# facebookresearch/PointContrast

Measured on AMD Instinct MI355X. Metric: scene-pairs/sec, ScanNet 2.5cm Res16UNet34C PointInfoNCE, higher is better.
Workload: dtype f32; 1 GPU; BASELINE configs[1]: Res16UNet34C, nce loss, voxel 0.025 m, 4 pairs/GPU, 87380+87371 active voxels per forward pair on rank 0, npos 4096, T 0.4, SGD(lr 0.1, mom 0.8, wd 1e-4); global_batch=4, parallelism=dp1, engine=native, pair_execution=one two-segment pass (BatchNorm statistics per cloud)

## Files before the change

pointcontrast_amd/csrc/common.h:

```cpp
#pragma once
#include <hip/hip_runtime.h>
#include <stdarg.h>
#include <stdint.h>
#include <stdio.h>

#include "../../include/pcmi.h"

namespace pcmi {

void set_error(const char* fmt, ...);

#define PCMI_HIP_CHECK(expr)                                                             \
  do {                                                                                   \
    hipError_t _e = (expr);                                                              \
    if (_e != hipSuccess) {                                                              \
      pcmi::set_error("%s:%d: %s -> %s", __FILE__, __LINE__, #expr, hipGetErrorString(_e)); \
      return PCMI_ERR_HIP;                                                               \
    }                                                                                    \
  } while (0)

#define PCMI_REQUIRE(cond, code, ...)  \
  do {                                 \
    if (!(cond)) {                     \
      pcmi::set_error(__VA_ARGS__);    \
      return (code);                   \
    }                                  \
  } while (0)

extern thread_local long g_launches;
#define PCMI_LAUNCH_CHECK()         \
  do {                              \
    ++pcmi::g_launches;             \
    PCMI_HIP_CHECK(hipGetLastError()); \
  } while (0)

static inline hipStream_t as_stream(pcmi_stream_t s) { return reinterpret_cast<hipStream_t>(s); }

static inline int64_t ceil_div(int64_t a, int64_t b) { return (a + b - 1) / b; }
static inline size_t align_up(size_t a, size_t b) { return (a + b - 1) / b * b; }

constexpr uint64_t kEmptyKey = ~0ull;
constexpr int kCoordBias = 1 << 17;

__host__ __device__ inline uint64_t pack_key(int b, int x, int y, int z) {
  return ((uint64_t)(uint32_t)b << 54) | ((uint64_t)(uint32_t)(x + kCoordBias) << 36) |
         ((uint64_t)(uint32_t)(y + kCoordBias) << 18) | (uint64_t)(uint32_t)(z + kCoordBias);
}

__host__ __device__ inline uint32_t hash_key(uint64_t k) {
  k ^= k >> 33;
  k *= 0xff51afd7ed558ccdull;
  k ^= k >> 33;
  k *= 0xc4ceb9fe1a85ec53ull;
  k ^= k >> 33;
  return (uint32_t)k;
}

#if defined(__HIPCC__)
__device__ inline bool arrive_last(unsigned* counter, unsigned expected, unsigned* s_flag ) {
  __syncthreads();
  if (threadIdx.x == 0 && threadIdx.y == 0 && threadIdx.z == 0) {
    __builtin_amdgcn_fence(__ATOMIC_RELEASE, "agent");
    asm volatile("s_waitcnt vmcnt(0)" ::: "memory");
    const unsigned t = __hip_atomic_fetch_add(counter, 1u, __ATOMIC_RELAXED, __HIP_MEMORY_SCOPE_AGENT);
    const unsigned last = (t + 1u == expected) ? 1u : 0u;
    if (last) {
      __hip_atomic_store(counter, 0u, __ATOMIC_RELAXED, __HIP_MEMORY_SCOPE_AGENT);
      __builtin_amdgcn_fence(__ATOMIC_ACQUIRE, "agent");
    }
    *s_flag = last;
  }
  __syncthreads();
  return *s_flag != 0u;
}
#endif

__host__ __device__ inline int floor_div(int a, int d) {
  int q = a / d;
  return (a % d != 0 && ((a < 0) != (d < 0))) ? q - 1 : q;
}

}
```

pointcontrast_amd/csrc/spconv.hip:

```cpp
#include <algorithm>
#include <cmath>
#include <cstdlib>

#include "common.h"
#include "internal.h"
#include "spconv_args.h"
#include "spconv_plan.h"

namespace pcmi {

typedef float f32x16 __attribute__((ext_vector_type(16)));
typedef float v4f __attribute__((ext_vector_type(4)));

constexpr int kKC = 32;


template <int NT, bool WT, int KC = kKC>
__device__ __forceinline__ void load_b_regs(v4f (&breg)[NT * KC / 32], const float* __restrict__ wb, int64_t w_sc,
                                            int64_t w_sn, int c0, int n0, int t) {
  constexpr int NS = 32 * NT;
#pragma unroll
  for (int i = 0; i < NT * KC / 32; ++i) {
    const int e = t + i * 256;
    if (!WT) {
// ... 180 lines not shown
#pragma unroll
            for (int nt = 0; nt < NT; ++nt) bf[q % PF][nt] = sb[(8 * (qq >> 2) + (qq & 3)) * LDB + nt * 32];
          }
          __builtin_amdgcn_sched_barrier(0);
        }
      }
      if (more) store_b((step + 1) & 1);
      __syncthreads();
#pragma unroll
      for (int b = 0; b < BPG; ++b) a0[b] = a1[b];
      v0 = v1;
    }
  }

  if (KG > 1) {
    if (kg > 0) {
      float* red = s_f + ((kg - 1) * RW + rg) * 32 * NS;
#pragma unroll
      for (int nt = 0; nt < NT; ++nt)
#pragma unroll
        for (int j = 0; j < 16; ++j) {
          const int i = (j & 3) + 8 * (j >> 2) + 4 * h;
          red[i * NS + nt * 32 + r] = acc[nt][j];
        }
    }
    __syncthreads();
    if (kg == 0) {
#pragma unroll
      for (int g = 1; g < KG; ++g) {
        const float* red = s_f + ((g - 1) * RW + rg) * 32 * NS;
#pragma unroll
        for (int nt = 0; nt < NT; ++nt)
#pragma unroll
          for (int j = 0; j < 16; ++j) {
            const int i = (j & 3) + 8 * (j >> 2) + 4 * h;
            acc[nt][j] += red[i * NS + nt * 32 + r];
          }
      }
    }
  }

  if (kg == 0) {
    float* outp = a.out + (PAIR ? 0 : (int64_t)blockIdx.z * a.split_stride);
    float bv[NT];
#pragma unroll
    for (int nt = 0; nt < NT; ++nt) bv[nt] = a.bias ? a.bias[n0 + nt * 32 + r] : 0.f;
#pragma unroll
    for (int j = 0; j < 16; ++j) {
      const int i = (j & 3) + 8 * (j >> 2) + 4 * h;
      const int32_t orow = s_orow[rg * 32 + i];
      if (orow >= 0) {
        float* op = outp + (int64_t)orow * a.out_ld + n0 + r;
        if (a.accumulate) {
#pragma unroll
          for (int nt = 0; nt < NT; ++nt) op[nt * 32] += acc[nt][j] + bv[nt];
        } else {
#pragma unroll
          for (int nt = 0; nt < NT; ++nt) op[nt * 32] = acc[nt][j] + bv[nt];
        }
      }
    }
  }
}

typedef float f32x4 __attribute__((ext_vector_type(4)));
__host__ __device__ constexpr int kConv16Waves(int nt) { return nt <= 3 ? 4 : 3; }

template <int NT, bool WT, bool SK>
__global__ __launch_bounds__(256, kConv16Waves(NT)) void spconv16p_kernel(ConvArgs a) {
  constexpr int TM = 128, NS = 32 * NT, CTN = 2 * NT;
  constexpr int LDB = NS + 4;
  constexpr int KSLOTS = PCMI_MAX_KERNEL_VOLUME;
  constexpr uint32_t kAbsent = 0x80000000u;
  constexpr int kRsrcFlags = 0x00020000;
  __shared__ __attribute__((aligned(16))) float s_f[2 * kKC * LDB];
  __shared__ uint32_t s_off[KSLOTS][TM];
  __shared__ int32_t s_orow[TM];
  __shared__ int2 s_kmeta[KSLOTS];
  __shared__ int32_t s_kabs[KSLOTS];
  __shared__ int32_t s_nk;
  __shared__ int64_t s_tile[2];

  const int n0 = blockIdx.y * NS;
  int sk_g = 0, sk_tile = 0, sk_u = 0, sk_u1 = 0;
  bool sk_first = true;
  if constexpr (SK) {
    const int G = (int)gridDim.x;
    sk_g = (int)(blockIdx.x & 7) * (G / 8) + (int)(blockIdx.x >> 3);
    const int U = a.sk_pref[a.sk_tiles] * (a.C / kKC);
    const int per = (U + G - 1) / G;
    sk_u = sk_g * per;
    sk_u1 = min(U, sk_u + per);
    if (sk_u >= sk_u1) return;
    if (threadIdx.x < 64) {
      int lo = 0, n = a.sk_tiles;
      while (n > 1) {
        const int stride = (n + 63) / 64;
        const int probe = lo + (int)threadIdx.x * stride;
        const bool le = probe < lo + n && a.sk_pref[probe] * (a.C / kKC) <= sk_u;
        const int cnt = __popcll(__ballot(le));
        const int nlo = lo + max(cnt - 1, 0) * stride;
        n = min(stride, lo + n - nlo);
        lo = nlo;
      }
      if (threadIdx.x == 0) s_tile[0] = lo;
    }
    __syncthreads();
    sk_tile = __builtin_amdgcn_readfirstlane((int)s_tile[0]);
  }
  const __amdgpu_buffer_rsrc_t xr = __builtin_amdgcn_make_buffer_rsrc(const_cast<float*>(a.x), 0, 0x7FFFFFFF, kRsrcFlags);
  const __amdgpu_buffer_rsrc_t wr = __builtin_amdgcn_make_buffer_rsrc(const_cast<float*>(a.w), 0, 0x7FFFFFFF, kRsrcFlags);
  const uint32_t ld_bytes = (uint32_t)(a.x_ld * 4);
  const uint32_t wk_bytes = (uint32_t)(a.w_kstride * 4);
  const int sk_total = SK ? sk_u1 - sk_u : 0;
  int sk_done = 0, prio_qtr = -1;
  for (;;) {
  bool sk_whole = true;
  int sk_next_u = 0, sk_c0 = 0, sk_steps = 0;
  int t = threadIdx.x;
  if constexpr (SK) asm volatile("" : "+v"(t));
  const int lane = t & 63, wave = t >> 6;
  const int i = lane & 15, kk = lane >> 4;
  if constexpr (SK) {
    const int64_t row0 = (int64_t)sk_tile * TM;
    const uint32_t tmask = a.sk_mask[sk_tile];
    const int nch_ = a.C / kKC;
    const int pref = a.sk_pref[sk_tile] * nch_, ns_t = __popc(tmask) * nch_;
    const int jb = sk_u - pref, je = min(sk_u1 - pref, ns_t);
    sk_whole = (jb == 0 && je == ns_t);
    sk_next_u = pref + je;
    const int o0 = jb / nch_, o1 = (je - 1) / nch_;
    sk_c0 = jb - o0 * nch_;
    sk_steps = je - jb;
    if (t < a.K && ((tmask >> t) & 1u)) {
      const int j = __popc(tmask & ((1u << t) - 1u));
      if (j >= o0 && j <= o1) {
        s_kabs[j - o0] = t;
        s_kmeta[j - o0] = make_int2(j - o0, (int)((uint32_t)a.wsel[t] * wk_bytes));
      }
    }
    if (t == 0) s_nk = sk_steps > 0 ? o1 - o0 + 1 : 0;
    if (t < TM) s_orow[t] = (row0 + t < a.n_rows) ? (a.perm ? a.perm[row0 + t] : (int32_t)(row0 + t)) : -1;
    __syncthreads();
    const int cnt = sk_steps > 0 ? o1 - o0 + 1 : 0;
    for (int p = t; p < cnt * TM; p += 256) {
      const int q = p / TM, rr = p - q * TM;
      const int64_t row = row0 + rr;
      const int32_t v = row < a.n_rows ? a.nbr[(int64_t)s_kabs[q] * a.n_rows + row] : -1;
      s_off[q][rr] = v >= 0 ? (uint32_t)v * ld_bytes : kAbsent;
    }
  } else {
    int64_t tile = blockIdx.x;
    if (a.xcd_tiles > 0) {
      tile = (int64_t)(blockIdx.x & 7) * a.xcd_tiles + (blockIdx.x >> 3);
      if (tile * TM >= a.n_rows) return;
    }
    const int64_t row0 = tile * TM;
    const int kbeg = (int)((int64_t)a.K * blockIdx.z / a.ksplit);
    const int kend = (int)((int64_t)a.K * (blockIdx.z + 1) / a.ksplit);
    if (t < TM) s_orow[t] = (row0 + t < a.n_rows) ? (a.perm ? a.perm[row0 + t] : (int32_t)(row0 + t)) : -1;
    for (int p = t; p < (kend - kbeg) * TM; p += 256) {
      const int q = p / TM, rr = p - q * TM;
      const int64_t row = row0 + rr;
      int32_t v = -1;
      if (row < a.n_rows) v = a.nbr ? a.nbr[(int64_t)(kbeg + q) * a.n_rows + row] : (int32_t)row;
      s_off[q][rr] = v >= 0 ? (uint32_t)v * ld_bytes : kAbsent;
    }
    __syncthreads();
    if (t < 64) {
      int nk = 0;
      for (int q = 0; q < kend - kbeg; ++q) {
        bool any = false;
        for (int rr = t; rr < TM; rr += 64) any |= (s_off[q][rr] != kAbsent);
        if (__any(any)) {
          if (t == 0) s_kmeta[nk] = make_int2(q, (int)((uint32_t)a.wsel[kbeg + q] * wk_bytes));
// ... 50 lines not shown
    const uint32_t wofs = (uint32_t)__builtin_amdgcn_readfirstlane(l_meta.y);
    const char* row = reinterpret_cast<const char*>(&s_off[0][0]) + min(krow, KSLOTS - 1) * (TM * 4) + off_lane;
    l_voff[0] = *reinterpret_cast<const uint32_t*>(row);
    l_voff[1] = *reinterpret_cast<const uint32_t*>(row + 64);
    const uint32_t soff = (uint32_t)__builtin_amdgcn_readfirstlane((int)(wofs + (uint32_t)lc * b_chunk_bytes));
#pragma unroll
    for (int q = 0; q < NT; ++q)
      breg[q] = __builtin_bit_cast(v4f, __builtin_amdgcn_raw_buffer_load_b128(wr, live ? bvo[q] : kAbsent, live ? soff : 0u, 0));
  };
  auto stage_a = [&](v4f (&dst)[2][2], bool live) -> int {
    const uint32_t v0 = live ? l_voff[0] : kAbsent, v1 = live ? l_voff[1] : kAbsent;
    const int va = (__any(v0 != kAbsent) ? 1 : 0) | (__any(v1 != kAbsent) ? 2 : 0);
    const uint32_t soff = (uint32_t)__builtin_amdgcn_readfirstlane(lc * (kKC * 4));
    const uint32_t o0 = v0 + 16 * kk, o1 = v1 + 16 * kk;
    dst[0][0] = __builtin_bit_cast(v4f, __builtin_amdgcn_raw_buffer_load_b128(xr, o0, soff, 0));
    dst[1][0] = __builtin_bit_cast(v4f, __builtin_amdgcn_raw_buffer_load_b128(xr, o1, soff, 0));
    dst[0][1] = __builtin_bit_cast(v4f, __builtin_amdgcn_raw_buffer_load_b128(xr, o0 + 64, soff, 0));
    dst[1][1] = __builtin_bit_cast(v4f, __builtin_amdgcn_raw_buffer_load_b128(xr, o1 + 64, soff, 0));
    return va;
  };

  if (nsteps > 0) {
    stage_meta();
    stage_b(true);
    va0 = stage_a(a0, true);
    store_b(0);
    __syncthreads();
    auto do_step = [&](int step, v4f (&cur)[2][2], int va_cur, v4f (&nxt)[2][2], int& va_nxt) {
      const bool more = step + 1 < nsteps;
      if constexpr (SK) {
        const int qtr = __builtin_amdgcn_readfirstlane(((sk_done + step) * 4) / max(sk_total, 1));
        if (qtr != prio_qtr) {
          prio_qtr = qtr;
          if (qtr <= 0) __builtin_amdgcn_s_setprio(3);
          else if (qtr == 1) __builtin_amdgcn_s_setprio(2);
          else if (qtr == 2) __builtin_amdgcn_s_setprio(1);
          else __builtin_amdgcn_s_setprio(0);
        }
      }
      const float* sb = s_f + (step & 1) * (kKC * LDB) + i + (4 * kk) * LDB;
      constexpr int QN = 8, PF = 2;
      float bf[PF][CTN];
      if (va_cur) {
#pragma unroll
        for (int q = 0; q < PF; ++q)
#pragma unroll
          for (int ct = 0; ct < CTN; ++ct) bf[q][ct] = sb[(16 * (q >> 2) + (q & 3)) * LDB + ct * 16];
      }
      __builtin_amdgcn_sched_barrier(0);
      const bool g0 = (va_cur & 1) != 0, g1 = (va_cur & 2) != 0;
#pragma unroll
      for (int q = 0; q < QN; ++q) {
        const float av0 = cur[0][q >> 2][q & 3], av1 = cur[1][q >> 2][q & 3];
        if (g0) {
#pragma unroll
          for (int ct = 0; ct < CTN; ++ct)
            acc[0][ct] = __builtin_amdgcn_mfma_f32_16x16x4f32(av0, bf[q % PF][ct], acc[0][ct], 0, 0, 0);
        }
        if (g1) {
#pragma unroll
          for (int ct = 0; ct < CTN; ++ct)
            acc[1][ct] = __builtin_amdgcn_mfma_f32_16x16x4f32(av1, bf[q % PF][ct], acc[1][ct], 0, 0, 0);
        }
        if (va_cur && q + PF < QN) {
          const int qq = q + PF;
#pragma unroll
          for (int ct = 0; ct < CTN; ++ct) bf[q % PF][ct] = sb[(16 * (qq >> 2) + (qq & 3)) * LDB + ct * 16];
        }
        if (q == 0) stage_meta();
        if (q == 1) stage_b(more);
        if (q == 2) va_nxt = stage_a(nxt, more);
        __builtin_amdgcn_sched_barrier(0);
      }
      if (more) store_b((step + 1) & 1);
      __syncthreads();
    };
    for (int step = 0; step < nsteps; step += 2) {
      do_step(step, a0, va0, a1, va1);
      if (step + 1 < nsteps) do_step(step + 1, a1, va1, a0, va0);
    }
  }

  if (SK && !sk_whole) {
    float* pp = a.sk_part + ((int64_t)(2 * sk_g + (sk_first ? 0 : 1)) * TM + wave * 32) * a.N + n0 + i;
#pragma unroll
    for (int g = 0; g < 2; ++g)
#pragma unroll
      for (int r = 0; r < 4; ++r) {
        const int rl = g * 16 + 4 * kk + r;
#pragma unroll
        for (int ct = 0; ct < CTN; ++ct) pp[(int64_t)rl * a.N + ct * 16] = acc[g][ct][r];
      }
  } else {
    float* outp = a.out + (int64_t)blockIdx.z * a.split_stride;
    float bv[CTN];
#pragma unroll
    for (int ct = 0; ct < CTN; ++ct) bv[ct] = a.bias ? a.bias[n0 + ct * 16 + i] : 0.f;
#pragma unroll
    for (int g = 0; g < 2; ++g)
#pragma unroll
      for (int r = 0; r < 4; ++r) {
        const int32_t orow = s_orow[wave * 32 + g * 16 + 4 * kk + r];
        if (orow >= 0) {
          float* op = outp + (int64_t)orow * a.out_ld + n0 + i;
          if (a.accumulate) {
#pragma unroll
            for (int ct = 0; ct < CTN; ++ct) op[ct * 16] += acc[g][ct][r] + bv[ct];
          } else {
#pragma unroll
            for (int ct = 0; ct < CTN; ++ct) op[ct * 16] = acc[g][ct][r] + bv[ct];
          }
        }
      }
  }
  if constexpr (!SK) {
    break;
  } else {
    sk_u = sk_next_u;
    ++sk_tile;
    sk_first = false;
    sk_done += nsteps;
    if (sk_u >= sk_u1) break;
    __syncthreads();
  }
  }
}

__global__ __launch_bounds__(256) void sk_fixup_kernel(const float* __restrict__ part, const int32_t* __restrict__ pref,
                                                       int n_tiles, int G, const int32_t* __restrict__ perm, int64_t n_rows,
                                                       int N, const float* __restrict__ bias, float* __restrict__ out,
                                                       int64_t out_ld, int accumulate, int sub) {
  constexpr int TM = 128;
  const int tile = blockIdx.x;
  const int U = pref[n_tiles] * sub, per = (U + G - 1) / G;
  const int u0 = pref[tile] * sub, u1 = pref[tile + 1] * sub;
  if (u1 <= u0) return;
  const int g_first = u0 / per, g_last = (u1 - 1) / per;
  if (g_first == g_last) return;
  const int n4 = N / 4;
  const int64_t row0 = (int64_t)tile * TM;
  for (int e = threadIdx.x; e < TM * n4; e += 256) {
    const int rr = e / n4, c = (e - rr * n4) * 4;
    const int64_t row = row0 + rr;
    if (row >= n_rows) continue;
    float4 sum = make_float4(0.f, 0.f, 0.f, 0.f);
    for (int g = g_first; g <= g_last; ++g) {
      const int slot = (u0 <= g * per) ? 0 : 1;
      const float4 v = *reinterpret_cast<const float4*>(part + ((int64_t)(2 * g + slot) * TM + rr) * N + c);
      sum.x += v.x;
      sum.y += v.y;
      sum.z += v.z;
      sum.w += v.w;
    }
    if (bias) {
      sum.x += bias[c];
      sum.y += bias[c + 1];
      sum.z += bias[c + 2];
      sum.w += bias[c + 3];
    }
    const int64_t orow = perm ? perm[row] : row;
    float4* dst = reinterpret_cast<float4*>(out + orow * out_ld + c);
    if (accumulate) {
      const float4 o = *dst;
      sum.x += o.x;
      sum.y += o.y;
      sum.z += o.z;
      sum.w += o.w;
    }
    *dst = sum;
  }
}

__global__ void split_reduce_kernel(const float* __restrict__ part, int64_t split_stride, int ksplit,
                                    int64_t n_rows, int N, const float* __restrict__ bias,
                                    float* __restrict__ out, int64_t out_ld, int accumulate) {
  const int64_t idx = (int64_t)blockIdx.x * blockDim.x + threadIdx.x;
  const int n4 = N / 4;
  if (idx >= n_rows * n4) return;
  const int64_t row = idx / n4;
  const int c = (int)(idx % n4) * 4;
  float4 s = make_float4(0.f, 0.f, 0.f, 0.f);
  for (int i0 = 0; i0 < ksplit; i0 += 8) {
    float4 v[8];
#pragma unroll
    for (int u = 0; u < 8; ++u)
      v[u] = i0 + u < ksplit ? *reinterpret_cast<const float4*>(part + (int64_t)(i0 + u) * split_stride + row * N + c)
                             : make_float4(0.f, 0.f, 0.f, 0.f);
#pragma unroll
    for (int u = 0; u < 8; ++u) {
      s.x += v[u].x;
      s.y += v[u].y;
      s.z += v[u].z;
      s.w += v[u].w;
    }
  }
  if (bias) {
    s.x += bias[c];
    s.y += bias[c + 1];
    s.z += bias[c + 2];
    s.w += bias[c + 3];
  }
  float4* dst = reinterpret_cast<float4*>(out + row * out_ld + c);
  if (accumulate) {
    const float4 o = *dst;
    s.x += o.x;
    s.y += o.y;
    s.z += o.z;
    s.w += o.w;
  }
  *dst = s;
}

template <int CIN>
__global__ __launch_bounds__(256) void stem_fwd_kernel(const float* __restrict__ x, int64_t x_ld,
                                                       const float* __restrict__ w, int cout,
                                                       const int32_t* __restrict__ nbr, int K,
                                                       int64_t n_rows, const float* __restrict__ bias,
                                                       float* __restrict__ out, int64_t out_ld) {
  extern __shared__ float s_w[];
  for (int i = threadIdx.x; i < K * CIN * cout; i += 256) s_w[i] = w[i];
  __syncthreads();
  const int rows_per_block = 256 / 32;
  const int n = threadIdx.x & 31;
  const int64_t row = (int64_t)blockIdx.x * rows_per_block + (threadIdx.x >> 5);
  if (row >= n_rows) return;
  for (int nn = n; nn < cout; nn += 32) {
    float acc = bias ? bias[nn] : 0.f;
    for (int k = 0; k < K; ++k) {
      const int32_t idx = nbr ? nbr[(int64_t)k * n_rows + row] : (int32_t)row;
      if (idx < 0) continue;
      const float* xp = x + (int64_t)idx * x_ld;
#pragma unroll
      for (int c = 0; c < CIN; ++c) acc = fmaf(xp[c], s_w[(k * CIN + c) * cout + nn], acc);
    }
    out[row * out_ld + nn] = acc;
  }
}

template <int K>
__global__ __launch_bounds__(256) void stem32_fwd_kernel(const float* __restrict__ x, int64_t x_ld,
                                                         const float* __restrict__ w ,
                                                         const int32_t* __restrict__ nbr, int64_t n_rows,
                                                         const float* __restrict__ bias, float* __restrict__ out,
                                                         int64_t out_ld) {
  const int64_t row = (int64_t)blockIdx.x * 256 + threadIdx.x;
  if (row >= n_rows) return;
  int32_t idx[K];
#pragma unroll
  for (int k = 0; k < K; ++k) idx[k] = nbr ? nbr[(int64_t)k * n_rows + row] : (int32_t)row;
  float xv[K][3];
#pragma unroll
  for (int k = 0; k < K; ++k) {
    const float* xp = x + (int64_t)max(idx[k], 0) * x_ld;
    const bool ok = idx[k] >= 0;
// ... 81 lines not shown
  const ConvPlan p = plan_conv(conv_env(), rows, 0, C, N, K, PCMI_CONV_FORM_TABLE);
  return p.kernel == PCMI_CONV_KERNEL_TABLE_X3 ? p.NT : 0;
}

static int run_gathered(const float* x, int64_t x_ld, int64_t x_rows, int C, const float* w, int cin, int cout,
                        bool w_transposed, int N, const pcmi_kmap_t* map, bool pair_mode,
                        bool swap_pairs, const int32_t* wsel, const float* bias, float* out,
                        int64_t out_ld, int64_t n_rows, int accumulate, void* ws, size_t ws_bytes,
                        hipStream_t st) {
  PCMI_REQUIRE(C % 32 == 0 && N % 32 == 0, PCMI_ERR_UNSUPPORTED,
               "spconv: channels (%d -> %d) must be multiples of 32 on the MFMA path", C, N);
  PCMI_REQUIRE(x_ld % 4 == 0 && out_ld >= N && out_ld % 4 == 0 && ((uintptr_t)x % 16 == 0) && ((uintptr_t)w % 16 == 0) &&
                   ((uintptr_t)out % 16 == 0),
               PCMI_ERR_INVALID, "spconv: operands must be 16-byte aligned with ld %% 4 == 0");
  if (n_rows == 0) return PCMI_OK;
  ConvArgs a = {};
  a.x = x;
  a.x_ld = x_ld;
  a.C = C;
  a.w = w;
  a.w_kstride = (int64_t)cin * cout;
  if (!w_transposed) {
    a.w_sc = cout;
    a.w_sn = 1;
  } else {
    a.w_sc = 1;
    a.w_sn = cout;
  }
  a.N = N;
  a.K = map ? map->K : 1;
  for (int k = 0; k < PCMI_MAX_KERNEL_VOLUME; ++k) a.wsel[k] = wsel ? wsel[k] : k;
  a.n_rows = n_rows;
  a.bias = bias;
  a.nbr = !map || pair_mode ? nullptr : map->nbr;
  a.ksplit = 1;
  a.accumulate = accumulate;
  a.out = out;
  a.out_ld = out_ld;
  int form = !map ? PCMI_CONV_FORM_NONE : pair_mode ? PCMI_CONV_FORM_PAIRS : PCMI_CONV_FORM_TABLE;
  if (form == PCMI_CONV_FORM_TABLE && map->perm && map->nbr_perm) {
    a.nbr = map->nbr_perm;
    a.perm = map->perm;
    if (map->tile_pref && map->n_tiles == ceil_div(n_rows, 128)) form = PCMI_CONV_FORM_TABLE_UNITS;
  }
  const ConvPlan p = plan_conv(conv_env(), n_rows, x_rows * x_ld * 4, C, N, a.K, form);
  PCMI_REQUIRE(p.ws_bytes == 0 || (ws && ws_bytes >= p.ws_bytes), PCMI_ERR_WORKSPACE, "spconv: workspace %zu < %zu bytes",
               ws_bytes, p.ws_bytes);
  const int terms = conv_terms();
  if (p.pack_bytes) {
    a.wpack = x3_find_prepacked(w, w_transposed, p.NT, terms);
    if (!a.wpack) {
      a.wpack = (char*)ws + p.pack_offset;
      const int rc_pack = x3_pack_weights(a, p.NT, const_cast<void*>(a.wpack), st, terms);
      if (rc_pack) return rc_pack;
    }
  }
  int rc;
  switch (p.kernel) {
    case PCMI_CONV_KERNEL_PAIR: {
      a.pair_src = swap_pairs ? map->pair_in : map->pair_out;
      a.pair_dst = swap_pairs ? map->pair_out : map->pair_in;
      a.offs = map->offs;
      const int TM = 32 * p.RW;
      int64_t tiles = 0;
      if (map->M >= 0)
        for (int k = 0; k < a.K; ++k) tiles += ceil_div(map->offs_host[k + 1] - map->offs_host[k], TM);
      else
        tiles = ceil_div(kmap_pairs_bound(*map), TM) + a.K;
      if (tiles == 0) return PCMI_OK;
      dim3 grid((unsigned)tiles, (unsigned)(N / (32 * p.NT)), 1);
      return w_transposed ? launch_rw<true, true>(p.RW, p.NT, a, grid, st) : launch_rw<false, true>(p.RW, p.NT, a, grid, st);
    }
    case PCMI_CONV_KERNEL_32R:
      return conv32r_launch(w_transposed, a, st);
    case PCMI_CONV_KERNEL_UNITS_16:
    case PCMI_CONV_KERNEL_UNITS_X3: {
      const bool x3 = p.kernel == PCMI_CONV_KERNEL_UNITS_X3;
      const int G = x3 ? x3_workgroups(p.NT, terms) : sk_workgroups(p.NT);
      a.sk_mask = map->tile_mask;
      a.sk_pref = map->tile_pref;
      a.sk_tiles = (int)map->n_tiles;
      a.sk_part = (float*)ws;
      dim3 grid((unsigned)G, (unsigned)(N / (32 * p.NT)), 1);
      if (x3)
        rc = x3_launch(p.NT, true, a, grid, st, terms);
      else
        rc = w_transposed ? launch16<true, true>(p.NT, a, grid, st) : launch16<false, true>(p.NT, a, grid, st);
      if (rc) return rc;
      const int sub = C / kKC;
      sk_fixup_kernel<<<dim3((unsigned)a.sk_tiles), 256, 0, st>>>(a.sk_part, a.sk_pref, a.sk_tiles, G, a.perm, n_rows, N, bias,
                                                                out, out_ld, accumulate, sub);
      PCMI_LAUNCH_CHECK();
      return PCMI_OK;
    }
  }
  if (p.ksplit > 1) {
    a.ksplit = p.ksplit;
    a.split_stride = n_rows * N;
    a.out = (float*)ws;
    a.out_ld = N;
    a.bias = nullptr;
    a.accumulate = 0;
  }
  int64_t tiles = ceil_div(n_rows, 32 * p.RW);
  if (tiles >= 64) {
    a.xcd_tiles = (int)ceil_div(tiles, 8);
    tiles = (int64_t)a.xcd_tiles * 8;
  }
  dim3 grid((unsigned)tiles, (unsigned)(N / (32 * p.NT)), (unsigned)p.ksplit);
  switch (p.kernel) {
    case PCMI_CONV_KERNEL_TABLE_X3: rc = x3_launch(p.NT, false, a, grid, st, terms); break;
    case PCMI_CONV_KERNEL_TABLE_16:
      rc = w_transposed ? launch16<true, false>(p.NT, a, grid, st) : launch16<false, false>(p.NT, a, grid, st);
      break;
    case PCMI_CONV_KERNEL_DEEP: rc = w_transposed ? launch_deep<true>(p.NT, a, grid, st) : launch_deep<false>(p.NT, a, grid, st); break;
    default: rc = w_transposed ? launch_rw<true, false>(p.RW, p.NT, a, grid, st) : launch_rw<false, false>(p.RW, p.NT, a, grid, st);
  }
  if (rc) return rc;
  if (p.ksplit > 1) {
    const int64_t n4 = n_rows * (N / 4);
    split_reduce_kernel<<<dim3((unsigned)ceil_div(n4, 256)), 256, 0, st>>>((const float*)ws, a.split_stride, p.ksplit,
                                                                         n_rows, N, bias, out, out_ld, accumulate);
    PCMI_LAUNCH_CHECK();
  }
  return PCMI_OK;
}

size_t spconv_fwd_bwd_workspace(int64_t n_in, int64_t n_out, int cin, int cout, int K) {
  const ConvEnv env = conv_env();
  auto split = [&](int64_t rows, int C, int N) -> size_t {
    if (rows <= 0 || C % 32 != 0 || N % 32 != 0) return 0;
    return std::max(plan_conv(env, rows, 0, C, N, K, PCMI_CONV_FORM_TABLE).split_bytes,
                    plan_conv(env, rows, INT64_MAX, C, N, K, PCMI_CONV_FORM_TABLE).split_bytes);
  };
  const size_t ks = std::max(split(n_out, cin, cout), split(n_in, cout, cin));
  const size_t sk = n_in == n_out ? std::max(sk_partial_bytes(env, n_out, cout, K), sk_partial_bytes(env, n_in, cin, K)) : 0;
  const size_t pack = (K > 1 && cin % 32 == 0 && cout % 32 == 0) ? x3_pack_bytes(K, cin, cout) : 0;
  return align_up(std::max(ks, sk), 256) + pack;
}

}

namespace pcmi {

int spconv_forward_m32(const float* in, int64_t in_ld, int64_t n_in, int cin, const float* weight, int cout,
                       const pcmi_kmap_t* map, int transpose, const float* bias, float* out, int64_t out_ld,
                       int64_t n_out, int accumulate, void* ws, size_t ws_bytes, hipStream_t st) {
  PCMI_REQUIRE(in && weight && out && cin > 0 && cout > 0, PCMI_ERR_INVALID, "spconv_fwd: null/empty argument");
  if (map) {
    const int64_t mi = transpose ? map->n_out : map->n_in, mo = transpose ? map->n_in : map->n_out;
    PCMI_REQUIRE(mi == n_in && mo == n_out, PCMI_ERR_INVALID, "spconv_fwd: rows (%lld -> %lld) do not match the map (%lld -> %lld)",
                 (long long)n_in, (long long)n_out, (long long)mi, (long long)mo);
  } else {
    PCMI_REQUIRE(n_in == n_out, PCMI_ERR_INVALID, "spconv_fwd: dense path needs n_in == n_out");
  }
  if (cin < 8) {
    PCMI_REQUIRE(cin == 3 && !transpose && !accumulate && (!map || map->stride == 1), PCMI_ERR_UNSUPPORTED,
                 "spconv_fwd: cin=%d only supported as the 3-channel stride-1 stem", cin);
    if (n_out == 0) return PCMI_OK;
    const int K = map ? map->K : 1;
    if (cout == 32 && K == 27 && out_ld % 4 == 0 && (uintptr_t)out % 16 == 0) {
      stem32_fwd_kernel<27><<<dim3((unsigned)ceil_div(n_out, 256)), 256, 0, st>>>(in, in_ld, weight, map->nbr, n_out, bias, out,
                                                                                 out_ld);
      PCMI_LAUNCH_CHECK();
      return PCMI_OK;
    }
    const size_t lds = sizeof(float) * K * 3 * cout;
    stem_fwd_kernel<3><<<dim3((unsigned)ceil_div(n_out, 8)), 256, lds, st>>>(in, in_ld, weight, cout, map ? map->nbr : nullptr,
                                                                            K, n_out, bias, out, out_ld);
    PCMI_LAUNCH_CHECK();
    return PCMI_OK;
  }
  const bool pair_mode = map && transpose;
  PCMI_REQUIRE(!(map && transpose && map->stride != 2), PCMI_ERR_UNSUPPORTED, "spconv_fwd: transposed conv needs a stride-2 map");
  return run_gathered(in, in_ld, n_in, cin, weight, cin, cout, false, cout, map, pair_mode, false, nullptr, bias, out,
                      out_ld, n_out, accumulate, ws, ws_bytes, st);
// ... 74 lines not shown
```

pointcontrast_amd/csrc/spconv_args.h:

```cpp
#pragma once
#include "common.h"

namespace pcmi {

struct ConvArgs {
  const float* x;
  int64_t x_ld;
  int C;
  const float* w;
  int64_t w_kstride;
  int64_t w_sc, w_sn;
  int N;
  const int32_t* nbr;
  const int32_t* perm;
  const int32_t* pair_src;
  const int32_t* pair_dst;
  const int64_t* offs;
  int K;
  int32_t wsel[PCMI_MAX_KERNEL_VOLUME];
  int64_t n_rows;
  float* out;
  int64_t out_ld;
  int64_t split_stride;
  int ksplit;
  const float* bias;
  int xcd_tiles;
  int accumulate;
  const uint32_t* sk_mask;
  const int32_t* sk_pref;
  int sk_tiles;
  float* sk_part;
  const void* wpack;
};

size_t x3_pack_bytes(int K, int C, int N);
int x3_pack_weights(const ConvArgs& a, int NT, void* out, hipStream_t st, int terms);
int x3_launch(int NT, bool sk, const ConvArgs& a, dim3 grid, hipStream_t st, int terms);
int x3_workgroups(int NT, int terms);
int x3_plan_nt(int64_t rows, int C, int N, int K);

bool conv32r_eligible(int64_t min_rows, int64_t rows, int64_t x_bytes, int C, int N, int K, bool table);
int conv32r_launch(bool w_transposed, const ConvArgs& a, hipStream_t st);

struct X3PackJob {
  const float* w;
  int64_t w_kstride, w_sc, w_sn;
  int K, C, N, NS;
  int terms;
  void* out;
  int64_t first_item;
};
int x3_pack_many(const X3PackJob* jobs_dev, int n_jobs, int64_t total_items, hipStream_t st, int64_t first_item = 0);
struct X3Prepacked {
  const float* w;
  int transposed;
  int NT;
  int terms;
  const void* pack;
};
void x3_set_prepacked(const X3Prepacked* table, int n);
const void* x3_find_prepacked(const float* w, bool transposed, int NT, int terms);

}
```

pointcontrast_amd/csrc/spconv_x3.hip:

```cpp
#include <algorithm>
#include <cstdio>
#include <cstdlib>

#include "common.h"
#include "internal.h"
#include "spconv_args.h"
#include "x3_split.h"

namespace pcmi {

__host__ __device__ constexpr int x3_piece(int n, int kk) { return (n >> 4) * 64 + kk * 16 + (n & 15); }

__host__ __device__ constexpr int x3_channel(int kk, int e) { return 4 * kk + (e & 3) + 16 * (e >> 2); }

template <int TERMS>
__global__ __launch_bounds__(256) void x3_pack_kernel(const float* __restrict__ w, int64_t w_kstride, int64_t w_sc, int64_t w_sn,
                                                      int K, int C, int N, int NS, u32x4* __restrict__ out) {
  const int nch = C / kKC, nns = N / NS;
  const int64_t total = (int64_t)K * nch * nns * NS * 4;
  const int64_t idx = (int64_t)blockIdx.x * 256 + threadIdx.x;
  if (idx >= total) return;
  const int kk = (int)(idx & 3);
  int64_t r = idx >> 2;
  const int nl = (int)(r % NS);
// ... 7 lines not shown
#pragma unroll
  for (int e = 0; e < 4; ++e) {
    x0[e] = wb[(int64_t)(cc * kKC + x3_channel(kk, e)) * w_sc];
    x1[e] = wb[(int64_t)(cc * kKC + x3_channel(kk, e + 4)) * w_sc];
  }
  u32x4 h, m, l;
  split_terms<TERMS>(x0, x1, h, m, l);
  u32x4* blk = out + (((int64_t)wk * nch + cc) * nns + ns) * (TERMS * NS * 4);
  const int piece = x3_piece(nl, kk);
  blk[0 * NS * 4 + piece] = h;
  if constexpr (TERMS == 3) {
    blk[1 * NS * 4 + piece] = m;
    blk[2 * NS * 4 + piece] = l;
  }
}

__global__ __launch_bounds__(256) void x3_pack_many_kernel(const X3PackJob* __restrict__ jobs, int n_jobs, int64_t total,
                                                           int64_t item0) {
  const int64_t idx = item0 + (int64_t)blockIdx.x * 256 + threadIdx.x;
  if (idx >= total) return;
  int lo = 0, hi = n_jobs - 1;
  while (lo < hi) {
    const int mid = (lo + hi + 1) >> 1;
    if (jobs[mid].first_item <= idx) lo = mid; else hi = mid - 1;
  }
  const X3PackJob jb = jobs[lo];
  const int64_t loc = idx - jb.first_item;
  const int nch = jb.C / kKC, nns = jb.N / jb.NS;
  const int kk = (int)(loc & 3);
  int64_t r = loc >> 2;
  const int nl = (int)(r % jb.NS);
  r /= jb.NS;
  const int ns = (int)(r % nns);
  r /= nns;
  const int cc = (int)(r % nch);
  const int wk = (int)(r / nch);
  const float* wb = jb.w + (int64_t)wk * jb.w_kstride + (int64_t)(ns * jb.NS + nl) * jb.w_sn;
  v4f x0, x1;
#pragma unroll
  for (int e = 0; e < 4; ++e) {
    x0[e] = wb[(int64_t)(cc * kKC + x3_channel(kk, e)) * jb.w_sc];
    x1[e] = wb[(int64_t)(cc * kKC + x3_channel(kk, e + 4)) * jb.w_sc];
  }
  const int piece = x3_piece(nl, kk);
  if (jb.terms == 1) {
    u32x4 h;
    split1(x0, x1, h);
    reinterpret_cast<u32x4*>(jb.out)[(((int64_t)wk * nch + cc) * nns + ns) * (jb.NS * 4) + piece] = h;
    return;
  }
  u32x4 h, m, l;
  split3(x0, x1, h, m, l);
  u32x4* blk = reinterpret_cast<u32x4*>(jb.out) + (((int64_t)wk * nch + cc) * nns + ns) * (3 * jb.NS * 4);
  blk[0 * jb.NS * 4 + piece] = h;
  blk[1 * jb.NS * 4 + piece] = m;
  blk[2 * jb.NS * 4 + piece] = l;
}

template <int TERMS>
constexpr int x3_min_waves(int NT) { return TERMS == 3 ? (NT == 4 ? 2 : 3) : (NT == 2 ? 4 : 3); }
template <int NT, bool SK, bool DMA, int TERMS>
__global__ __launch_bounds__(256, x3_min_waves<TERMS>(NT)) void spconv16x_kernel(ConvArgs a) {
  constexpr int TM = 128, NS = 32 * NT, CTN = 2 * NT;
  constexpr int KSLOTS = PCMI_MAX_KERNEL_VOLUME;
  constexpr uint32_t kAbsent = 0x80000000u;
  constexpr int kRsrcFlags = 0x00020000;
  constexpr int PIECES = TERMS * NS * 4;
  constexpr int BLOCK_BYTES = PIECES * 16;
  constexpr int BR = (PIECES + 255) / 256;
  static_assert(CTN >= 3, "the three load stages sit behind the MFMAs of column tiles 0, 1, 2");
  __shared__ __attribute__((aligned(16))) u32x4 s_b[2][PIECES];
  __shared__ uint32_t s_off[KSLOTS][TM];
  __shared__ int32_t s_orow[TM];
  __shared__ int2 s_kmeta[KSLOTS];
  __shared__ int32_t s_kabs[KSLOTS];
  __shared__ int32_t s_nk;
  __shared__ int64_t s_tile[2];

  const int n0 = blockIdx.y * NS;
  const int nch = a.C / kKC;
  const uint32_t chunk_bytes = (uint32_t)gridDim.y * BLOCK_BYTES;
  const uint32_t wk_bytes = (uint32_t)nch * chunk_bytes;
  const uint32_t slice_bytes = (uint32_t)blockIdx.y * BLOCK_BYTES;
  int sk_g = 0, sk_tile = 0, sk_u = 0, sk_u1 = 0;
  bool sk_first = true;
  if constexpr (SK) {
    const int G = (int)gridDim.x;
    sk_g = (int)(blockIdx.x & 7) * (G / 8) + (int)(blockIdx.x >> 3);
    const int U = a.sk_pref[a.sk_tiles] * nch;
    const int per = (U + G - 1) / G;
    sk_u = sk_g * per;
    sk_u1 = min(U, sk_u + per);
    if (sk_u >= sk_u1) return;
    if (threadIdx.x < 64) {
      int lo = 0, n = a.sk_tiles;
      while (n > 1) {
        const int stride = (n + 63) / 64;
        const int probe = lo + (int)threadIdx.x * stride;
        const bool le = probe < lo + n && a.sk_pref[probe] * nch <= sk_u;
        const int cnt = __popcll(__ballot(le));
        const int nlo = lo + max(cnt - 1, 0) * stride;
        n = min(stride, lo + n - nlo);
        lo = nlo;
      }
      if (threadIdx.x == 0) s_tile[0] = lo;
    }
    __syncthreads();
    sk_tile = __builtin_amdgcn_readfirstlane((int)s_tile[0]);
  }
  const __amdgpu_buffer_rsrc_t xr = __builtin_amdgcn_make_buffer_rsrc(const_cast<float*>(a.x), 0, 0x7FFFFFFF, kRsrcFlags);
  const __amdgpu_buffer_rsrc_t wr = __builtin_amdgcn_make_buffer_rsrc(const_cast<void*>(a.wpack), 0, 0x7FFFFFFF, kRsrcFlags);
  const uint32_t ld_bytes = (uint32_t)(a.x_ld * 4);
  const int sk_total = SK ? sk_u1 - sk_u : 0;
  int sk_done = 0, prio_qtr = -1;
  for (;;) {
  bool sk_whole = true;
  int sk_next_u = 0, sk_c0 = 0, sk_steps = 0;
  int t = threadIdx.x;
  if constexpr (SK) asm volatile("" : "+v"(t));
  const int lane = t & 63, wave = t >> 6;
  const int i = lane & 15, kk = lane >> 4;
  if constexpr (SK) {
    const int64_t row0 = (int64_t)sk_tile * TM;
    const uint32_t tmask = a.sk_mask[sk_tile];
    const int pref = a.sk_pref[sk_tile] * nch, ns_t = __popc(tmask) * nch;
    const int jb = sk_u - pref, je = min(sk_u1 - pref, ns_t);
    sk_whole = (jb == 0 && je == ns_t);
    sk_next_u = pref + je;
    const int o0 = jb / nch, o1 = (je - 1) / nch;
    sk_c0 = jb - o0 * nch;
    sk_steps = je - jb;
    if (t < a.K && ((tmask >> t) & 1u)) {
      const int j = __popc(tmask & ((1u << t) - 1u));
      if (j >= o0 && j <= o1) {
        s_kabs[j - o0] = t;
        s_kmeta[j - o0] = make_int2(j - o0, (int)((uint32_t)a.wsel[t] * wk_bytes + slice_bytes));
      }
    }
    if (t == 0) s_nk = sk_steps > 0 ? o1 - o0 + 1 : 0;
    if (t < TM) s_orow[t] = (row0 + t < a.n_rows) ? (a.perm ? a.perm[row0 + t] : (int32_t)(row0 + t)) : -1;
    __syncthreads();
    const int cnt = sk_steps > 0 ? o1 - o0 + 1 : 0;
    {
      const int rr = t & (TM - 1);
      const int64_t row = row0 + rr;
      const bool row_ok = row < a.n_rows;
      const int64_t row_c = row_ok ? row : a.n_rows - 1;
      for (int q0 = t >> 7; q0 < cnt; q0 += 8) {
        int32_t v[4];
#pragma unroll
        for (int u = 0; u < 4; ++u) v[u] = a.nbr[(int64_t)s_kabs[min(q0 + 2 * u, cnt - 1)] * a.n_rows + row_c];
#pragma unroll
        for (int u = 0; u < 4; ++u)
          if (q0 + 2 * u < cnt) s_off[q0 + 2 * u][rr] = (row_ok && v[u] >= 0) ? (uint32_t)v[u] * ld_bytes : kAbsent;
      }
    }
  } else {
    int64_t tile = blockIdx.x;
    if (a.xcd_tiles > 0) {
      tile = (int64_t)(blockIdx.x & 7) * a.xcd_tiles + (blockIdx.x >> 3);
      if (tile * TM >= a.n_rows) return;
    }
    const int64_t row0 = tile * TM;
    const int kbeg = (int)((int64_t)a.K * blockIdx.z / a.ksplit);
    const int kend = (int)((int64_t)a.K * (blockIdx.z + 1) / a.ksplit);
    if (t < TM) s_orow[t] = (row0 + t < a.n_rows) ? (a.perm ? a.perm[row0 + t] : (int32_t)(row0 + t)) : -1;
    for (int p = t; p < (kend - kbeg) * TM; p += 256) {
      const int q = p / TM, rr = p - q * TM;
      const int64_t row = row0 + rr;
      int32_t v = -1;
      if (row < a.n_rows) v = a.nbr ? a.nbr[(int64_t)(kbeg + q) * a.n_rows + row] : (int32_t)row;
      s_off[q][rr] = v >= 0 ? (uint32_t)v * ld_bytes : kAbsent;
    }
    __syncthreads();
    if (t < 64) {
// ... 87 lines not shown
    dst[1][1] = __builtin_bit_cast(v4f, __builtin_amdgcn_raw_buffer_load_b128(xr, o1 + 64, soff, 0));
    return va;
  };

  if (nsteps > 0) {
    stage_meta();
    stage_b(true, 0);
    va0 = stage_a(a0, true);
    store_b(0);
    __syncthreads();
    auto do_step = [&](int step, v4f (&cur)[2][2], int va_cur, v4f (&nxt)[2][2], int& va_nxt) {
      const bool more = step + 1 < nsteps;
      if constexpr (SK) {
        const int qtr = __builtin_amdgcn_readfirstlane(((sk_done + step) * 4) / max(sk_total, 1));
        if (qtr != prio_qtr) {
          prio_qtr = qtr;
          if (qtr <= 0) __builtin_amdgcn_s_setprio(3);
          else if (qtr == 1) __builtin_amdgcn_s_setprio(2);
          else if (qtr == 2) __builtin_amdgcn_s_setprio(1);
          else __builtin_amdgcn_s_setprio(0);
        }
      }
      const bool g0 = (va_cur & 1) != 0, g1 = (va_cur & 2) != 0;
      u32x4 ah[2], am[2], al[2];
      if (g0) split_terms<TERMS>(cur[0][0], cur[0][1], ah[0], am[0], al[0]);
      if (g1) split_terms<TERMS>(cur[1][0], cur[1][1], ah[1], am[1], al[1]);
      const u32x4* sb = &s_b[step & 1][kk * 16 + i];
      u32x4 bh[2], bm[2], bl[2];
      if (va_cur) {
        bh[0] = sb[0 * NS * 4];
        if constexpr (TERMS == 3) {
          bm[0] = sb[1 * NS * 4];
          bl[0] = sb[2 * NS * 4];
        }
      }
      __builtin_amdgcn_sched_barrier(0);
#pragma unroll
      for (int ct = 0; ct < CTN; ++ct) {
        const int rb = ct & 1;
        if (va_cur && ct + 1 < CTN) {
          bh[rb ^ 1] = sb[(0 * NS + 16 * (ct + 1)) * 4];
          if constexpr (TERMS == 3) {
            bm[rb ^ 1] = sb[(1 * NS + 16 * (ct + 1)) * 4];
            bl[rb ^ 1] = sb[(2 * NS + 16 * (ct + 1)) * 4];
          }
        }
#define PCMI_X3_MFMA(G, AT, BT)                                                                                             \
  acc[G][ct] = __builtin_amdgcn_mfma_f32_16x16x32_bf16(__builtin_bit_cast(bf16x8, AT[G]), __builtin_bit_cast(bf16x8, BT[rb]), \
                                                       acc[G][ct], 0, 0, 0)
#define PCMI_X3_SIX(G)        \
  if constexpr (TERMS == 3) { \
    PCMI_X3_MFMA(G, al, bh);  \
    PCMI_X3_MFMA(G, ah, bl);  \
    PCMI_X3_MFMA(G, am, bm);  \
    PCMI_X3_MFMA(G, am, bh);  \
    PCMI_X3_MFMA(G, ah, bm);  \
  }                           \
  PCMI_X3_MFMA(G, ah, bh)
        if (g0 && g1) {
          PCMI_X3_SIX(0);
          PCMI_X3_SIX(1);
        } else if (g0) {
          PCMI_X3_SIX(0);
        } else if (g1) {
          PCMI_X3_SIX(1);
        }
#undef PCMI_X3_SIX
#undef PCMI_X3_MFMA
        if (ct == 0) stage_meta();
        if (ct == 1) stage_b(more, (step + 1) & 1);
        if (ct == 2) va_nxt = stage_a(nxt, more);
        __builtin_amdgcn_sched_barrier(0);
      }
      if (more) store_b((step + 1) & 1);
      __syncthreads();
    };
    for (int step = 0; step < nsteps; step += 2) {
      do_step(step, a0, va0, a1, va1);
      if (step + 1 < nsteps) do_step(step + 1, a1, va1, a0, va0);
    }
  }

  if (SK && !sk_whole) {
    float* pp = a.sk_part + ((int64_t)(2 * sk_g + (sk_first ? 0 : 1)) * TM + wave * 32) * a.N + n0 + i;
#pragma unroll
    for (int g = 0; g < 2; ++g)
#pragma unroll
      for (int r = 0; r < 4; ++r) {
        const int rl = g * 16 + 4 * kk + r;
#pragma unroll
        for (int ct = 0; ct < CTN; ++ct) pp[(int64_t)rl * a.N + ct * 16] = acc[g][ct][r];
      }
  } else {
    float* outp = a.out + (int64_t)blockIdx.z * a.split_stride;
    float bv[CTN];
#pragma unroll
    for (int ct = 0; ct < CTN; ++ct) bv[ct] = a.bias ? a.bias[n0 + ct * 16 + i] : 0.f;
#pragma unroll
    for (int g = 0; g < 2; ++g)
#pragma unroll
      for (int r = 0; r < 4; ++r) {
        const int32_t orow = s_orow[wave * 32 + g * 16 + 4 * kk + r];
        if (orow >= 0) {
          float* op = outp + (int64_t)orow * a.out_ld + n0 + i;
          if (a.accumulate) {
#pragma unroll
            for (int ct = 0; ct < CTN; ++ct) op[ct * 16] += acc[g][ct][r] + bv[ct];
          } else {
#pragma unroll
            for (int ct = 0; ct < CTN; ++ct) op[ct * 16] = acc[g][ct][r] + bv[ct];
          }
        }
      }
  }
  if constexpr (!SK) {
    break;
  } else {
    sk_u = sk_next_u;
    ++sk_tile;
    sk_first = false;
    sk_done += nsteps;
    if (sk_u >= sk_u1) break;
    __syncthreads();
  }
  }
}

template <bool SK, bool DMA, int TERMS>
static int launch_x3(int NT, const ConvArgs& a, dim3 grid, hipStream_t st) {
  switch (NT) {
    case 2: spconv16x_kernel<2, SK, DMA, TERMS><<<grid, 256, 0, st>>>(a); break;
    case 3: spconv16x_kernel<3, SK, DMA, TERMS><<<grid, 256, 0, st>>>(a); break;
    case 4: spconv16x_kernel<4, SK, DMA, TERMS><<<grid, 256, 0, st>>>(a); break;
    default: set_error("spconv x3: bad NT %d", NT); return PCMI_ERR_INVALID;
  }
  PCMI_LAUNCH_CHECK();
  return PCMI_OK;
}

size_t x3_pack_bytes(int K, int C, int N) { return align_up((size_t)std::max(K, 1) * C * N * 6, 256); }

int x3_workgroups(int NT, int terms) {
  return (terms == 1 ? x3_min_waves<1>(NT) : x3_min_waves<3>(NT)) * num_cu() / 8 * 8;
}

int x3_pack_weights(const ConvArgs& a, int NT, void* out, hipStream_t st, int terms) {
  PCMI_REQUIRE(out && ((uintptr_t)out % 16 == 0) && a.C % kKC == 0 && a.N % (32 * NT) == 0 && (terms == 1 || terms == 3),
               PCMI_ERR_INVALID, "spconv x3: bad pack arguments (%d -> %d, NT %d, %d terms)", a.C, a.N, NT, terms);
  const int64_t total = (int64_t)a.K * (a.C / kKC) * a.N * 4;
  const dim3 grid((unsigned)ceil_div(total, 256));
  if (terms == 1)
    x3_pack_kernel<1><<<grid, 256, 0, st>>>(a.w, a.w_kstride, a.w_sc, a.w_sn, a.K, a.C, a.N, 32 * NT, reinterpret_cast<u32x4*>(out));
  else
    x3_pack_kernel<3><<<grid, 256, 0, st>>>(a.w, a.w_kstride, a.w_sc, a.w_sn, a.K, a.C, a.N, 32 * NT, reinterpret_cast<u32x4*>(out));
  PCMI_LAUNCH_CHECK();
  return PCMI_OK;
}

int x3_pack_many(const X3PackJob* jobs_dev, int n_jobs, int64_t total_items, hipStream_t st, int64_t first_item) {
  if (n_jobs <= 0 || total_items <= first_item) return PCMI_OK;
  x3_pack_many_kernel<<<dim3((unsigned)ceil_div(total_items - first_item, 256)), 256, 0, st>>>(jobs_dev, n_jobs, total_items, first_item);
  PCMI_LAUNCH_CHECK();
  return PCMI_OK;
}

static thread_local const X3Prepacked* t_prepacked = nullptr;
static thread_local int t_n_prepacked = 0;
void x3_set_prepacked(const X3Prepacked* table, int n) {
  t_prepacked = table;
  t_n_prepacked = table ? n : 0;
}
const void* x3_find_prepacked(const float* w, bool transposed, int NT, int terms) {
  for (int i = 0; i < t_n_prepacked; ++i)
    if (t_prepacked[i].w == w && (t_prepacked[i].transposed != 0) == transposed && t_prepacked[i].NT == NT &&
        t_prepacked[i].terms == terms)
// ... 13 lines not shown
```

Baseline: 291.7 scene-pairs/sec.

## Fuse stream-K fixup into conv kernel via last-arriving block reduction

Replaces the separate stream-K fixup kernel with an in-kernel epilogue. Each block writes its partial tile, then bumps a per-tile atomic counter, and the last contributor sums all partials, adds bias and writes (or accumulates into) the output rows. This removes one kernel launch per stream-K conv and the extra pass over partials, at the cost of atomics, fences and a serialized reduction tail inside the conv kernel. It also needs per-stream counter buffers.

```diff
diff --git a/pointcontrast_amd/csrc/common.h b/pointcontrast_amd/csrc/common.h
--- a/pointcontrast_amd/csrc/common.h
+++ b/pointcontrast_amd/csrc/common.h
@@ -73,6 +73,23 @@
   __syncthreads();
   return *s_flag != 0u;
 }
+
+__device__ inline bool arrive_last_wt(unsigned* counter, unsigned expected, unsigned* s_flag ) {
+  asm volatile("s_waitcnt vmcnt(0)" ::: "memory");
+  __syncthreads();
+  if (threadIdx.x == 0 && threadIdx.y == 0 && threadIdx.z == 0) {
+    const unsigned t = __hip_atomic_fetch_add(counter, 1u, __ATOMIC_RELAXED, __HIP_MEMORY_SCOPE_AGENT);
+    const unsigned last = (t + 1u == expected) ? 1u : 0u;
+    if (last) {
+      __hip_atomic_store(counter, 0u, __ATOMIC_RELAXED, __HIP_MEMORY_SCOPE_AGENT);
+      __builtin_amdgcn_fence(__ATOMIC_ACQUIRE, "agent");
+      asm volatile("s_waitcnt vmcnt(0)" ::: "memory");
+    }
+    *s_flag = last;
+  }
+  __syncthreads();
+  return *s_flag != 0u;
+}
 #endif
 
 __host__ __device__ inline int floor_div(int a, int d) {
diff --git a/pointcontrast_amd/csrc/spconv.hip b/pointcontrast_amd/csrc/spconv.hip
--- a/pointcontrast_amd/csrc/spconv.hip
+++ b/pointcontrast_amd/csrc/spconv.hip
@@ -286,15 +286,15 @@
   __shared__ int64_t s_tile[2];
 
   const int n0 = blockIdx.y * NS;
-  int sk_g = 0, sk_tile = 0, sk_u = 0, sk_u1 = 0;
+  int sk_g = 0, sk_tile = 0, sk_u = 0, sk_u1 = 0, sk_per = 1;
   bool sk_first = true;
   if constexpr (SK) {
     const int G = (int)gridDim.x;
     sk_g = (int)(blockIdx.x & 7) * (G / 8) + (int)(blockIdx.x >> 3);
     const int U = a.sk_pref[a.sk_tiles] * (a.C / kKC);
-    const int per = (U + G - 1) / G;
-    sk_u = sk_g * per;
-    sk_u1 = min(U, sk_u + per);
+    sk_per = (U + G - 1) / G;
+    sk_u = sk_g * sk_per;
+    sk_u1 = min(U, sk_u + sk_per);
     if (sk_u >= sk_u1) return;
     if (threadIdx.x < 64) {
       int lo = 0, n = a.sk_tiles;
@@ -511,15 +511,7 @@
   }
 
   if (SK && !sk_whole) {
-    float* pp = a.sk_part + ((int64_t)(2 * sk_g + (sk_first ? 0 : 1)) * TM + wave * 32) * a.N + n0 + i;
-#pragma unroll
-    for (int g = 0; g < 2; ++g)
-#pragma unroll
-      for (int r = 0; r < 4; ++r) {
-        const int rl = g * 16 + 4 * kk + r;
-#pragma unroll
-        for (int ct = 0; ct < CTN; ++ct) pp[(int64_t)rl * a.N + ct * 16] = acc[g][ct][r];
-      }
+    sk_piece_epilogue<CTN, 4>(*sk_kernarg<ConvArgs>(), acc, t, sk_g, sk_first, sk_tile, nch, sk_per, n0, s_orow, reinterpret_cast<unsigned*>(&s_tile[1]));
   } else {
     float* outp = a.out + (int64_t)blockIdx.z * a.split_stride;
     float bv[CTN];
@@ -555,50 +547,6 @@
   }
 }
 
-__global__ __launch_bounds__(256) void sk_fixup_kernel(const float* __restrict__ part, const int32_t* __restrict__ pref,
-                                                       int n_tiles, int G, const int32_t* __restrict__ perm, int64_t n_rows,
-                                                       int N, const float* __restrict__ bias, float* __restrict__ out,
-                                                       int64_t out_ld, int accumulate, int sub) {
-  constexpr int TM = 128;
-  const int tile = blockIdx.x;
-  const int U = pref[n_tiles] * sub, per = (U + G - 1) / G;
-  const int u0 = pref[tile] * sub, u1 = pref[tile + 1] * sub;
-  if (u1 <= u0) return;
-  const int g_first = u0 / per, g_last = (u1 - 1) / per;
-  if (g_first == g_last) return;
-  const int n4 = N / 4;
-  const int64_t row0 = (int64_t)tile * TM;
-  for (int e = threadIdx.x; e < TM * n4; e += 256) {
-    const int rr = e / n4, c = (e - rr * n4) * 4;
-    const int64_t row = row0 + rr;
-    if (row >= n_rows) continue;
-    float4 sum = make_float4(0.f, 0.f, 0.f, 0.f);
-    for (int g = g_first; g <= g_last; ++g) {
-      const int slot = (u0 <= g * per) ? 0 : 1;
-      const float4 v = *reinterpret_cast<const float4*>(part + ((int64_t)(2 * g + slot) * TM + rr) * N + c);
-      sum.x += v.x;
-      sum.y += v.y;
-      sum.z += v.z;
-      sum.w += v.w;
-    }
-    if (bias) {
-      sum.x += bias[c];
-      sum.y += bias[c + 1];
-      sum.z += bias[c + 2];
-      sum.w += bias[c + 3];
-    }
-    const int64_t orow = perm ? perm[row] : row;
-    float4* dst = reinterpret_cast<float4*>(out + orow * out_ld + c);
-    if (accumulate) {
-      const float4 o = *dst;
-      sum.x += o.x;
-      sum.y += o.y;
-      sum.z += o.z;
-      sum.w += o.w;
-    }
-    *dst = sum;
-  }
-}
 
 __global__ void split_reduce_kernel(const float* __restrict__ part, int64_t split_stride, int ksplit,
                                     int64_t n_rows, int N, const float* __restrict__ bias,
@@ -846,16 +794,10 @@
       a.sk_tiles = (int)map->n_tiles;
       a.sk_part = (float*)ws;
       dim3 grid((unsigned)G, (unsigned)(N / (32 * p.NT)), 1);
-      if (x3)
-        rc = x3_launch(p.NT, true, a, grid, st, terms);
-      else
-        rc = w_transposed ? launch16<true, true>(p.NT, a, grid, st) : launch16<false, true>(p.NT, a, grid, st);
-      if (rc) return rc;
-      const int sub = C / kKC;
-      sk_fixup_kernel<<<dim3((unsigned)a.sk_tiles), 256, 0, st>>>(a.sk_part, a.sk_pref, a.sk_tiles, G, a.perm, n_rows, N, bias,
-                                                                out, out_ld, accumulate, sub);
-      PCMI_LAUNCH_CHECK();
-      return PCMI_OK;
+      a.sk_cnt = stream_counters(st, (size_t)a.sk_tiles * grid.y);
+      if (!a.sk_cnt) return PCMI_ERR_HIP;
+      if (x3) return x3_launch(p.NT, true, a, grid, st, terms);
+      return w_transposed ? launch16<true, true>(p.NT, a, grid, st) : launch16<false, true>(p.NT, a, grid, st);
     }
   }
   if (p.ksplit > 1) {
diff --git a/pointcontrast_amd/csrc/spconv_args.h b/pointcontrast_amd/csrc/spconv_args.h
--- a/pointcontrast_amd/csrc/spconv_args.h
+++ b/pointcontrast_amd/csrc/spconv_args.h
@@ -30,8 +30,106 @@
   const int32_t* sk_pref;
   int sk_tiles;
   float* sk_part;
+  unsigned* sk_cnt;
   const void* wpack;
 };
+
+#if defined(__HIPCC__)
+template <typename A>
+__device__ __forceinline__ const __attribute__((address_space(4))) A* sk_kernarg() {
+  auto p = (const __attribute__((address_space(4))) A*)__builtin_amdgcn_kernarg_segment_ptr();
+  asm volatile("" : "+s"(p));
+  return p;
+}
+
+template <int CTN, int B, typename V4, typename Args>
+__device__ __forceinline__ void sk_piece_epilogue(const Args& a, const V4 (&acc)[2][CTN], int t, int sk_g, bool sk_first,
+                                                  int tile, int sub, int per, int n0, const int32_t* s_orow, unsigned* s_flag) {
+  constexpr int TM = 128, NS = 16 * CTN, N4S = NS / 4;
+  constexpr int EPT = TM * N4S / 256;
+  static_assert(EPT % B == 0, "the sum walks a thread's float4 in batches of B");
+  const int lane = t & 63, wave = t >> 6, i = lane & 15, kk = lane >> 4;
+  const __amdgpu_buffer_rsrc_t pr = __builtin_amdgcn_make_buffer_rsrc(
+      a.sk_part + (int64_t)(2 * sk_g + (sk_first ? 0 : 1)) * TM * a.N, 0, TM * a.N * 4, 0x00020000);
+  const uint32_t po = (uint32_t)((wave * 32 + 4 * kk) * a.N + n0 + i) * 4u;
+#pragma unroll
+  for (int g = 0; g < 2; ++g)
+#pragma unroll
+    for (int r = 0; r < 4; ++r) {
+      const uint32_t ro = po + (uint32_t)((g * 16 + r) * a.N) * 4u;
+#pragma unroll
+      for (int ct = 0; ct < CTN; ++ct)
+        __builtin_amdgcn_raw_buffer_store_b32(__builtin_bit_cast(uint32_t, (float)acc[g][ct][r]), pr, ro + ct * 64u, 0, 16);
+    }
+  asm volatile("" : "+s"(per));
+  const int u0 = a.sk_pref[tile] * sub, u1 = a.sk_pref[tile + 1] * sub;
+  const int g_first = u0 / per, g_last = (u1 - 1) / per;
+  if (!arrive_last_wt(a.sk_cnt + (tile * (a.N / NS) + n0 / NS), (unsigned)(g_last - g_first + 1), s_flag)) return;
+  const bool has_bias = a.bias != nullptr;
+  const bool accumulate = a.accumulate != 0;
+  for (int e0 = 0; e0 < EPT; e0 += B) {
+    int rr[B], c[B];
+    float4 sum[B];
+#pragma unroll
+    for (int u = 0; u < B; ++u) {
+      const int e = t + 256 * (e0 + u);
+      rr[u] = e / N4S;
+      c[u] = n0 + (e - rr[u] * N4S) * 4;
+      sum[u] = make_float4(0.f, 0.f, 0.f, 0.f);
+    }
+    for (int g = g_first; g <= g_last; ++g) {
+      const int slot = (u0 <= g * per) ? 0 : 1;
+      const float* ps = a.sk_part + (int64_t)(2 * g + slot) * TM * a.N;
+      float4 v[B];
+#pragma unroll
+      for (int u = 0; u < B; ++u) v[u] = *reinterpret_cast<const float4*>(ps + (int64_t)rr[u] * a.N + c[u]);
+#pragma unroll
+      for (int u = 0; u < B; ++u) {
+        sum[u].x += v[u].x;
+        sum[u].y += v[u].y;
+        sum[u].z += v[u].z;
+        sum[u].w += v[u].w;
+      }
+    }
+    if (has_bias) {
+      float b[B][4];
+#pragma unroll
+      for (int u = 0; u < B; ++u)
+#pragma unroll
+        for (int k = 0; k < 4; ++k) b[u][k] = a.bias[c[u] + k];
+#pragma unroll
+      for (int u = 0; u < B; ++u) {
+        sum[u].x += b[u][0];
+        sum[u].y += b[u][1];
+        sum[u].z += b[u][2];
+        sum[u].w += b[u][3];
+      }
+    }
+    int32_t orow[B];
+    float4* dst[B];
+#pragma unroll
+    for (int u = 0; u < B; ++u) {
+      orow[u] = s_orow[rr[u]];
+      dst[u] = reinterpret_cast<float4*>(a.out + (int64_t)max(orow[u], 0) * a.out_ld + c[u]);
+    }
+    if (accumulate) {
+      float4 o[B];
+#pragma unroll
+      for (int u = 0; u < B; ++u) o[u] = *dst[u];
+#pragma unroll
+      for (int u = 0; u < B; ++u) {
+        sum[u].x += o[u].x;
+        sum[u].y += o[u].y;
+        sum[u].z += o[u].z;
+        sum[u].w += o[u].w;
+      }
+    }
+#pragma unroll
+    for (int u = 0; u < B; ++u)
+      if (orow[u] >= 0) *dst[u] = sum[u];
+  }
+}
+#endif
 
 size_t x3_pack_bytes(int K, int C, int N);
 int x3_pack_weights(const ConvArgs& a, int NT, void* out, hipStream_t st, int terms);
diff --git a/pointcontrast_amd/csrc/spconv_x3.hip b/pointcontrast_amd/csrc/spconv_x3.hip
--- a/pointcontrast_amd/csrc/spconv_x3.hip
+++ b/pointcontrast_amd/csrc/spconv_x3.hip
@@ -113,15 +113,15 @@
   const uint32_t chunk_bytes = (uint32_t)gridDim.y * BLOCK_BYTES;
   const uint32_t wk_bytes = (uint32_t)nch * chunk_bytes;
   const uint32_t slice_bytes = (uint32_t)blockIdx.y * BLOCK_BYTES;
-  int sk_g = 0, sk_tile = 0, sk_u = 0, sk_u1 = 0;
+  int sk_g = 0, sk_tile = 0, sk_u = 0, sk_u1 = 0, sk_per = 1;
   bool sk_first = true;
   if constexpr (SK) {
     const int G = (int)gridDim.x;
     sk_g = (int)(blockIdx.x & 7) * (G / 8) + (int)(blockIdx.x >> 3);
     const int U = a.sk_pref[a.sk_tiles] * nch;
-    const int per = (U + G - 1) / G;
-    sk_u = sk_g * per;
-    sk_u1 = min(U, sk_u + per);
+    sk_per = (U + G - 1) / G;
+    sk_u = sk_g * sk_per;
+    sk_u1 = min(U, sk_u + sk_per);
     if (sk_u >= sk_u1) return;
     if (threadIdx.x < 64) {
       int lo = 0, n = a.sk_tiles;
@@ -375,15 +375,8 @@
   }
 
   if (SK && !sk_whole) {
-    float* pp = a.sk_part + ((int64_t)(2 * sk_g + (sk_first ? 0 : 1)) * TM + wave * 32) * a.N + n0 + i;
-#pragma unroll
-    for (int g = 0; g < 2; ++g)
-#pragma unroll
-      for (int r = 0; r < 4; ++r) {
-        const int rl = g * 16 + 4 * kk + r;
-#pragma unroll
-        for (int ct = 0; ct < CTN; ++ct) pp[(int64_t)rl * a.N + ct * 16] = acc[g][ct][r];
-      }
+    constexpr int SB = (TERMS == 3 && NT >= 3) ? 2 * NT : 4;
+    sk_piece_epilogue<CTN, SB>(*sk_kernarg<ConvArgs>(), acc, t, sk_g, sk_first, sk_tile, nch, sk_per, n0, s_orow, reinterpret_cast<unsigned*>(&s_tile[1]));
   } else {
     float* outp = a.out + (int64_t)blockIdx.z * a.split_stride;
     float bv[CTN];
```

Result: no change. 292.6 scene-pairs/sec, median of 6 (+0.3%).
